# amcpherson/remixt

Measured on AMD Instinct MI355X. Metric: EM iterations/sec (50k seg x 165 states), higher is better.
Workload: dtype f64

## Files before the change

### include/remixt_amd.h

```cpp
#ifndef REMIXT_AMD_H
#define REMIXT_AMD_H

#include <stdint.h>

#ifdef __cplusplus
extern "C" {
#endif

#define RMX_OK 0
#define RMX_EVALUE 1
#define RMX_EASSERT 2
#define RMX_EDEVICE 3
#define RMX_EUNSUPPORTED 4
#define RMX_EARG 5

#define RMX_MAX_CLONES 4

typedef struct rmx_batch rmx_batch;

typedef struct rmx_problem {
    int32_t num_clones;
    int32_t num_segments;
    int32_t num_breakpoints;
    int32_t num_cn_states;
// ... 58 lines not shown
    RMX_OPT_SEARCH_MODE,
    RMX_OPT_ELL_DENSE,
    RMX_OPT_STRIP,
    RMX_OPT_CELL_CACHE,
    RMX_OPT_SPARSE_TRIAL,
    RMX_OPT_FB_DEBUG,
    RMX_OPT_PAIRWISE_KERNEL,
    RMX_OPT_PACE_SWEEPS,
    RMX_OPT_FB_WG_BUDGET,
    RMX_OPT_TRIAL_KERNEL,
    RMX_OPT_GRAD_KERNEL,
    RMX_OPT_STREAM_POOL,
    RMX_OPT_VITERBI_CLUSTER,
    RMX_OPT_TRACEBACK,
    RMX_OPT_LT_CLASSES,
    RMX_OPT_COUNT
};
int rmx_set_default_option(int32_t option_id, int32_t value);
int rmx_set_option(rmx_batch *b, int32_t option_id, int32_t value);
int rmx_get_option(rmx_batch *b, int32_t option_id, int32_t *value);

int rmx_set_param(rmx_batch *b, int32_t r, int32_t param_id, double value);
int rmx_get_param(rmx_batch *b, int32_t r, int32_t param_id, double *value);
int rmx_set_transition_model(rmx_batch *b, int32_t model);
int rmx_set_array(rmx_batch *b, int32_t r, int32_t array_id, const void *host_src);
int rmx_get_array(rmx_batch *b, int32_t r, int32_t array_id, void *host_dst);
int rmx_fetch_indicators(rmx_batch *b, int32_t r0, int32_t r1, const double **total, const double **allele);
int rmx_calculate_log_transmat(rmx_batch *b, int32_t r, double *dst);
int rmx_weighted_search(const double *p, int64_t n, const double *u, int32_t k, int64_t *out, int64_t *positive);
int rmx_weighted_sample_round(const double *w, int64_t n, int64_t stride, double norm, const double *u, int32_t k,
// ... 106 lines not shown
```

### remixt_amd/bpmodel.py

```python
import ctypes as C

import numpy as np

from . import _lib

_dp = C.POINTER(C.c_double)
_ip = C.POINTER(C.c_int64)
_i32p = C.POINTER(C.c_int32)

RMX_EVALUE, RMX_EASSERT, RMX_EDEVICE, RMX_EUNSUPPORTED, RMX_EARG = 1, 2, 3, 4, 5

MAX_CLONES = 4
PARAM_IDS = {
    'negbin_r_0': 0, 'negbin_r_1': 1, 'negbin_hdel_mu': 2, 'negbin_hdel_r_0': 3, 'negbin_hdel_r_1': 4,
    'betabin_M_0': 5, 'betabin_M_1': 6, 'betabin_loh_p': 7, 'betabin_loh_M_0': 8, 'betabin_loh_M_1': 9,
    'prior_outlier_total': 10, 'prior_outlier_allele': 11, 'divergence_weight': 12, 'hmm_log_norm_const': 13,
}
ARRAY_IDS = {
    'h': 0, 'p_breakpoint': 1, 'p_allele_swap': 2, 'p_outlier_total': 3, 'p_outlier_allele': 4,
    'posterior_marginals': 5, 'framelogprob': 6, 'total_likelihood_mask': 7, 'allele_likelihood_mask': 8,
    'log_transmat': 9, 'cached_log_transmat': 10, 'joint_posterior_marginals': 11, 'state_sequence': 12,
}
_WRITABLE = {'h', 'p_breakpoint', 'p_allele_swap', 'p_outlier_total', 'p_outlier_allele', 'posterior_marginals',
             'total_likelihood_mask', 'allele_likelihood_mask'}
_STATE_TABLES = {'cn_states_total': 0, 'num_alleles_subclonal': 1, 'is_hdel': 2, 'is_loh': 3}


OPTION_IDS = dict((n, i) for i, n in enumerate((
    'fb_kernel', 'fb_nv', 'fb_breakend_codes', 'fuse_sweeps', 'two_streams', 'viterbi_plain', 'search_mode', 'ell_dense', 'strip',
    'cell_cache', 'sparse_trial', 'fb_debug', 'pairwise_kernel', 'pace_sweeps', 'fb_wg_budget', 'trial_kernel', 'grad_kernel', 'stream_pool', 'viterbi_cluster', 'traceback', 'lt_classes')))


def set_default_option(name, value):
    lib = _lib.load()
    rc = lib.rmx_set_default_option(OPTION_IDS[name], int(value))
    if rc:
        _raise(lib, rc)


def last_error_restarts():
    lib = _lib.load()
    n = lib.rmx_last_error_restarts(None, 0)
    if n <= 0:
        return []
    buf = (C.c_int32 * n)()
# ... 972 lines not shown
```

### remixt_amd/csrc/rmx_api.hip

```cpp
#include <hip/hip_runtime.h>
#include <algorithm>
#include <cmath>
#include <limits>
#include <atomic>
#include <cstdio>
#include <cstring>
#include <functional>
#include <map>
#include <mutex>
#include <string>
#include <vector>
#include <chrono>
#include <cstdlib>
#include <condition_variable>
#include <memory>

#include "rmx_kernels.h"
#include "rmx_host.h"

static thread_local std::string g_err;
static thread_local std::vector<int32_t> g_err_restarts;
static int fail(int code, const std::string &msg) { g_err = msg; g_err_restarts.clear(); return code; }
static int fail_flagged(int code, const std::string &msg) { g_err = msg; return code; }
static inline long long now_ns() { return std::chrono::duration_cast<std::chrono::nanoseconds>(std::chrono::steady_clock::now().time_since_epoch()).count(); }
// ... 25 lines not shown
    StreamPool &p = g_stream_pool[dev & 15];
    std::lock_guard<std::mutex> lk(p.mu);
    std::vector<hipStream_t> &idle = p.idle[role];
    if (!idle.empty()) { *out = idle.front(); idle.erase(idle.begin()); return RMX_OK; }
    if (hipStreamCreateWithFlags(out, hipStreamNonBlocking) != hipSuccess) return RMX_EDEVICE;
    p.created[role]++;
    return RMX_OK;
}
static void pool_release(int dev, int role, hipStream_t s) {
    hipStreamSynchronize(s);
    StreamPool &p = g_stream_pool[dev & 15];
    std::lock_guard<std::mutex> lk(p.mu);
    p.idle[role].push_back(s);
}

static int g_opt_default[RMX_OPT_COUNT] = {0, 0, 1, 1, 1, 0, 5, 0, 1, 1, 1, 0, 0, 0, 0, 0, 0, 1, 0, 0, 1};
static std::mutex g_opt_mu;

struct rmx_batch {
    hipEvent_t ev_pace = nullptr;
    int opt[RMX_OPT_COUNT];
    int device = 0;
    hipStream_t stream = nullptr;
    hipStream_t stream2 = nullptr;
    hipEvent_t ev_fb = nullptr, ev_brk = nullptr;
    bool own_stream = false, pooled_stream = false, pooled_stream2 = false;
    Dev d{};
    int R = 0;
    std::vector<int64_t> cn_classes;
    std::vector<int32_t> seg_class, brk_idx, brk_orient, tclass, brk_slot, be_n;
    std::vector<int64_t> brk_states, is_telomere;
    std::vector<std::pair<int, int>> tc_pairs;
    std::vector<double> Tsum;
    std::vector<RestartParams> rp;
    std::vector<char> tables_dirty, segc_dirty, ab_dirty;
    std::vector<double> segc_built;
    std::vector<char> sig_valid;
    std::vector<int> cache_stale;
    bool use_cache = false;
    std::vector<int> comp_dirty;
    std::vector<int> comp_base;
    std::vector<int> lt_valid;
    std::vector<int> lt_model, cached_model;
    double *Tval_m[2] = {nullptr, nullptr}; int8_t *af_m[2] = {nullptr, nullptr};
    std::vector<double> plain_T_init;
    std::vector<double> logZ;
    std::vector<char> logz_dirty;
    int *d_lt_valid = nullptr;
    double *d_partial = nullptr;
    double *d_be_e = nullptr;
    double *d_out4 = nullptr;
    double *d_ell_partial = nullptr;
    double *d_ell_out = nullptr;
    double *h_pinned = nullptr;
    hipEvent_t ev_copy = nullptr;
    double *h_ind = nullptr;
// ... 7 lines not shown
    int32_t *d_msample = nullptr, *d_mcounts = nullptr;
    std::vector<int> msample_count;
    double *d_mpartial = nullptr; size_t mpartial_cap = 0;
    std::vector<std::vector<int64_t>> sample_cache; std::vector<int> sample_count;
    double *d_grid_out = nullptr;
    GradFlatLayout gf_lay = {nullptr, nullptr, nullptr, nullptr};
    std::vector<double> gf_sig;
    std::vector<long long> sample_epoch, sig_epoch;
    int32_t *gf_nblk_host = nullptr;
    bool gf_first = false;
    unsigned *d_done = nullptr;
    int32_t *d_rlist = nullptr, *d_counts = nullptr; RestartParams *d_rp_stage = nullptr; double *d_batch_out = nullptr;
    void *h_batch = nullptr;
    std::vector<int32_t> plain_list; int32_t *d_plain_list = nullptr; double *d_plain_jt = nullptr;
    int last_search_blocks = 0;
    unsigned *d_vflag = nullptr; int cluster_timeouts = 0;
    int last_viterbi_wgs = 1;
    int32_t *d_vit_special = nullptr; int n_vit_special = -1;
    double *h_elbo = nullptr; hipEvent_t ev_elbo = nullptr; bool elbo_pending = false, elbo_sync = false; int elbo_r0 = 0, elbo_r1 = 0;
    double *d_vrow = nullptr; size_t vrow_cap = 0;
    uint16_t *d_bp = nullptr; double *d_final = nullptr; int64_t *d_path = nullptr; double *d_logprob = nullptr;
    std::vector<int64_t> last_path; int vit_cap = 0; size_t bp_cap = 0;
    int16_t *d_samp = nullptr; size_t samp_cap = 0; uint64_t *d_seeds = nullptr; uint32_t *d_sflags = nullptr;
    double *d_psum = nullptr; size_t psum_cap = 0; double *d_psw = nullptr; size_t psw_cap = 0;
    double *d_rgcw = nullptr; size_t rgcw_cap = 0;
    double *d_rgn = nullptr; size_t rgn_cap = 0; uint8_t *d_rgt = nullptr; size_t rgt_cap = 0; uint32_t *d_rflags = nullptr; int16_t *d_rgbp = nullptr; size_t rgbp_cap = 0; int kbest_lds_raised = 0;
    double *d_ovr = nullptr; size_t ovr_cap = 0; uint32_t *d_ovf = nullptr; size_t ovf_cap = 0; hipEvent_t ev_ov = nullptr;
    uint16_t *d_comp = nullptr; int32_t *d_ends = nullptr; size_t comp_cap = 0, ends_cap = 0; int last_traceback = 0;
    uint8_t *d_vit_code = nullptr; double *d_vit_val = nullptr; bool vit_code_ok = false, vit_mul_ok = false;
    FbLaunch fbG{}; size_t fbG_lds = 0;
// ... 397 lines not shown
            };
            if (!stale(r)) { r++; continue; }
            int e = r + 1;
            while (e < r1 && stale(e)) e++;
            { ProfScope ps(b, KID_SEG_CONST); hipLaunchKernelGGL(k_seg_const, dim3((b->d.N + 255) / 256, e - r), dim3(256), 0, b->stream, b->d, r); }
            for (int i = r; i < e; i++) b->segc_dirty[i] = 0;
            r = e;
        }
    }
    HIPCHK(hipGetLastError());
    return RMX_OK;
}
typedef void (*cells_kernel_t)(Dev, int);
template <int NS, int LTC> static cells_kernel_t cells_kernel_cached(int mode, int mask, int cache) {
    if (mode == 0) return cache == 2 ? k_cells<NS, 0, CM_ALL, 2, LTC> : k_cells<NS, 0, CM_ALL, 1, LTC>;
    if (mode == 1) return k_cells<NS, 1, CM_ALL, 2, LTC>;
    if (mode == 3) return k_cells<NS, 3, CM_ALL, 2, LTC>;
    if (cache == 2) return k_cells<NS, 2, 31, 2, LTC>;
    switch (mask) {
    case 1: return k_cells<NS, 2, 1, 1, LTC>; case 2: return k_cells<NS, 2, 2, 1, LTC>;
    case 3: return k_cells<NS, 2, 3, 1, LTC>; case 4: return k_cells<NS, 2, 4, 1, LTC>; case 8: return k_cells<NS, 2, 8, 1, LTC>;
    case 12: return k_cells<NS, 2, 12, 1, LTC>; case 15: return k_cells<NS, 2, 15, 1, LTC>; default: return k_cells<NS, 2, 31, 1, LTC>;
    }
}
template <int NS> static cells_kernel_t cells_kernel_ns(int mode, int mask, int cache, bool ltc) {
    if (cache) return ltc ? cells_kernel_cached<NS, 1>(mode, mask, cache) : cells_kernel_cached<NS, 0>(mode, mask, cache);
    if (mode == 0) return k_cells<NS, 0, CM_ALL, 0, 0>;
    if (mode == 1) return k_cells<NS, 1, CM_ALL, 0, 0>;
    switch (mask) {
    case 1: return k_cells<NS, 2, 1, 0, 0>; case 2: return k_cells<NS, 2, 2, 0, 0>;
    case 3: return k_cells<NS, 2, 3, 0, 0>; case 4: return k_cells<NS, 2, 4, 0, 0>; case 8: return k_cells<NS, 2, 8, 0, 0>;
    case 12: return k_cells<NS, 2, 12, 0, 0>; case 15: return k_cells<NS, 2, 15, 0, 0>; default: return k_cells<NS, 2, 31, 0, 0>;
    }
}
static bool use_strip(rmx_batch *b) { return b->d.S > 32 && b->d.S <= 384 && b->opt[RMX_OPT_STRIP]; }
static cells_kernel_t cells_kernel(rmx_batch *b, int mode, int mask, int cache) {
    const int ns = (b->d.S + 63) / 64;
    const bool ltc = cache != 0 && b->d.ltc != nullptr;
    switch (ns) { case 1: return cells_kernel_ns<1>(mode, mask, cache, ltc); case 2: return cells_kernel_ns<2>(mode, mask, cache, ltc);
                  case 3: return cells_kernel_ns<3>(mode, mask, cache, ltc); case 4: return cells_kernel_ns<4>(mode, mask, cache, ltc);
                  case 5: return cells_kernel_ns<5>(mode, mask, cache, ltc); default: return cells_kernel_ns<6>(mode, mask, cache, ltc); }
}
// ... 537 lines not shown
    HIPCHK(hipHostMalloc(&b->h_batch, (size_t)R * (sizeof(RestartParams) + 64) + 4096));
    HIPCHK(hipEventCreate(&b->tm_a)); HIPCHK(hipEventCreate(&b->tm_b));
    b->done_ev.resize(R);
    for (int r = 0; r < R; r++) HIPCHK(hipEventCreateWithFlags(&b->done_ev[r], hipEventDisableTiming));

    if ((rc = build_transitions(b))) { rmx_batch_destroy(b); return rc; }
    {
        double tmin = 0.;
        std::vector<double> tv((size_t)SS * d.TC);
        if (d.TC) HIPCHK(hipMemcpy(tv.data(), d.Tval, tv.size() * 8, hipMemcpyDeviceToHost));
        for (double v : tv) tmin = std::min(tmin, v);
        if (tmin < -650.) { rmx_batch_destroy(b); return fail(RMX_EUNSUPPORTED, "transition_log_prob * max copy-number change exceeds 650 nats: outside the linear-domain envelope"); }
    }

    b->sample_cache.assign(R, std::vector<int64_t>()); b->sample_count.assign(R, -1);
    b->rp.resize(R); b->tables_dirty.assign(R, 1); b->segc_dirty.assign(R, 1); b->ab_dirty.assign(R, 1); b->comp_dirty.assign(R, 31); b->comp_base.assign(R, 31); b->cache_stale.assign(R, 15); b->sig_valid.assign(R, 0); b->sample_epoch.assign(R, 0); b->sig_epoch.assign(R, 0); b->lt_valid.assign(R, 0); b->lt_model.assign(R, 0); b->cached_model.assign(R, 0); b->logZ.assign(R, 0.); b->logz_dirty.assign(R, 0);
    for (int r = 0; r < R; r++) {
        RestartParams &p = b->rp[r];
        memset(&p, 0, sizeof p);
        for (int m = 0; m < M; m++) p.h[m] = h_init[(size_t)r * M + m];
        p.p[RMX_P_NEGBIN_R_0] = 500.; p.p[RMX_P_NEGBIN_R_1] = 10.; p.p[RMX_P_NEGBIN_HDEL_MU] = 1e-5; p.p[RMX_P_NEGBIN_HDEL_R_0] = 10.;
        p.p[RMX_P_NEGBIN_HDEL_R_1] = 1.; p.p[RMX_P_BETABIN_M_0] = 500.; p.p[RMX_P_BETABIN_M_1] = 10.; p.p[RMX_P_BETABIN_LOH_P] = 1e-3;
        p.p[RMX_P_BETABIN_LOH_M_0] = 10.; p.p[RMX_P_BETABIN_LOH_M_1] = 1.; p.p[RMX_P_PRIOR_OUTLIER_TOTAL] = 0.01; p.p[RMX_P_PRIOR_OUTLIER_ALLELE] = 0.01;
        p.p[RMX_P_DIVERGENCE_WEIGHT] = std::fabs(divw[r]);
    }
    {
        std::vector<double> q2(RN * 2), v;
        for (size_t i = 0; i < RN; i++) { q2[2 * i] = 1. - 0.01; q2[2 * i + 1] = 0.01; }
        HIPCHK(hipMemcpy(d.qt, q2.data(), q2.size() * 8, hipMemcpyHostToDevice));
        HIPCHK(hipMemcpy(d.qa, q2.data(), q2.size() * 8, hipMemcpyHostToDevice));
        for (size_t i = 0; i < RN * 2; i++) q2[i] = 0.5;
// ... 64 lines not shown
    else { HIPCHK(hipStreamCreateWithFlags(&b->stream, hipStreamNonBlocking)); b->own_stream = true; }
    return RMX_OK;
}
int rmx_synchronize(rmx_batch *b) { BIND(b); HIPCHK(hipStreamSynchronize(b->stream)); return RMX_OK; }

int rmx_info(rmx_batch *b, int32_t what, int64_t *out) { BIND(b);
    switch (what) {
    case 0: *out = b->d.cn_max; break; case 1: *out = b->d.NC; break; case 2: *out = b->d.TC; break; case 3: *out = b->d.NBE; break;
    case 4: *out = b->d.SP; break; case 5: *out = b->fbv_rpt; break; case 6: *out = b->fbG.P; break; case 7: *out = b->fbG.NT; break;
    case 8: *out = b->fbG.BLK; break; case 9: *out = (int64_t)b->fbG_lds; break; case 10: *out = b->n_fast; break; case 11: *out = b->n_generic; break;
    case 60: *out = b->t_launch_ns; break; case 61: *out = b->t_wait_ns; break; case 62: *out = b->t_post_ns; break; case 63: *out = b->n_rounds; break;
    case 12: *out = b->last_fb_kernel; break; case 13: *out = b->last_fb_nv; break; case 14: *out = b->last_viterbi; break; case 15: *out = b->last_fb_nv_max; break;
    case 18: *out = b->last_viterbi_wgs; break; case 19: *out = b->last_traceback; break;
    case 64: *out = b->d.NT; break; case 65: *out = b->d.ltc ? 1 : 0; break;
    case 54: *out = b->cluster_timeouts; break;
    case 52: *out = b->last_search_blocks; break;
    case 16: { StreamPool &p_ = g_stream_pool[b->device & 15]; std::lock_guard<std::mutex> lk(p_.mu); *out = p_.created[0] + p_.created[1]; break; }
    case 17: { StreamPool &p_ = g_stream_pool[b->device & 15]; std::lock_guard<std::mutex> lk(p_.mu); *out = (int64_t)(p_.idle[0].size() + p_.idle[1].size()); break; }
    case 20: case 21: case 22: case 23: case 24: case 25: case 26: case 27: case 28: case 29: case 30: case 31: case 32: case 33: case 34: case 35: case 36: case 37: case 38: case 39:
    case 40: case 41: case 42: case 43: case 44: case 45: case 46: case 47: case 48: case 49: case 50: case 51:
        { if (!b->d_dbg) { *out = 0; break; } unsigned long long v[32]; HIPCHK(hipStreamSynchronize(b->stream)); HIPCHK(hipMemcpy(v, b->d_dbg, 256, hipMemcpyDeviceToHost)); *out = (int64_t)v[what - 20]; break; }
    default: return fail(RMX_EARG, "bad info id");
    }
    return RMX_OK;
}

static const int kParamComponents[RMX_P_HMM_LOG_NORM_CONST] = {CM_LT0, CM_LT1, CM_LT0 | CM_LT1, CM_LT0, CM_LT1, CM_LA0, CM_LA1, CM_LA0 | CM_LA1, CM_LA0, CM_LA1, 0, 0, 16};
int rmx_set_param(rmx_batch *b, int32_t r, int32_t id, double v) { BIND(b);
    if (r < 0 || r >= b->R || id < 0 || id >= RMX_P_HMM_LOG_NORM_CONST) return fail(RMX_EARG, "bad restart / param id");
    if (id == RMX_P_DIVERGENCE_WEIGHT) v = std::fabs(v);
// ... 24 lines not shown

static int array_shape(rmx_batch *b, int id, size_t *count, bool *is_int) {
    const Dev &d = b->d; *is_int = false;
    switch (id) {
    case RMX_A_H: *count = d.M; break;
    case RMX_A_P_BREAKPOINT: *count = (size_t)d.K * d.B; break;
    case RMX_A_P_ALLELE_SWAP: case RMX_A_P_OUTLIER_TOTAL: case RMX_A_P_OUTLIER_ALLELE: *count = (size_t)d.N * 2; break;
    case RMX_A_POSTERIOR_MARGINALS: case RMX_A_FRAMELOGPROB: *count = (size_t)d.N * d.S; break;
    case RMX_A_TOTAL_LIKELIHOOD_MASK: case RMX_A_ALLELE_LIKELIHOOD_MASK: case RMX_A_STATE_SEQUENCE: *count = d.N; *is_int = true; break;
    case RMX_A_LOG_TRANSMAT: case RMX_A_CACHED_LOG_TRANSMAT: case RMX_A_JOINT_POSTERIOR_MARGINALS: *count = (size_t)(d.N - 1) * d.S * d.S; break;
    default: return fail(RMX_EARG, "bad array id");
    }
    return RMX_OK;
}

int rmx_set_array(rmx_batch *b, int32_t r, int32_t id, const void *src) { BIND(b);
    if (r < 0 || r >= b->R || !src) return fail(RMX_EARG, "bad restart / null source");
    Dev &d = b->d;
    const size_t RN = (size_t)r * d.N;
    switch (id) {
    case RMX_A_H:
        for (int m = 0; m < d.M; m++) b->rp[r].h[m] = ((const double *)src)[m];
        b->tables_dirty[r] = 1; b->ab_dirty[r] = 1; b->comp_dirty[r] = 31; b->comp_base[r] = 31; b->cache_stale[r] = 15; return RMX_OK;
    case RMX_A_P_BREAKPOINT:
        if (d.K) HIPCHK(hipMemcpyAsync(d.pbrk + (size_t)r * d.K * d.B, src, (size_t)d.K * d.B * 8, hipMemcpyHostToDevice, b->stream));
        break;
    case RMX_A_P_ALLELE_SWAP: HIPCHK(hipMemcpyAsync(d.qs + RN * 2, src, (size_t)d.N * 16, hipMemcpyHostToDevice, b->stream)); break;
    case RMX_A_P_OUTLIER_TOTAL: HIPCHK(hipMemcpyAsync(d.qt + RN * 2, src, (size_t)d.N * 16, hipMemcpyHostToDevice, b->stream)); break;
    case RMX_A_P_OUTLIER_ALLELE: HIPCHK(hipMemcpyAsync(d.qa + RN * 2, src, (size_t)d.N * 16, hipMemcpyHostToDevice, b->stream)); break;
    case RMX_A_POSTERIOR_MARGINALS:
        HIPCHK(hipMemcpy2DAsync(d.post + RN * d.SP, (size_t)d.SP * 8, src, (size_t)d.S * 8, (size_t)d.S * 8, d.N, hipMemcpyHostToDevice, b->stream));
        b->ab_dirty[r] = 1; b->comp_dirty[r] = 31; b->comp_base[r] = 31; b->sig_valid[r] = 0; b->sig_epoch[r]++; break;
    case RMX_A_TOTAL_LIKELIHOOD_MASK: case RMX_A_ALLELE_LIKELIHOOD_MASK: {
        std::vector<uint8_t> m8(d.N);
        for (int n = 0; n < d.N; n++) m8[n] = ((const int64_t *)src)[n] != 0;
        HIPCHK(hipStreamSynchronize(b->stream));
        HIPCHK(hipMemcpy((void *)(id == RMX_A_TOTAL_LIKELIHOOD_MASK ? d.mask_t : d.mask_a), m8.data(), d.N, hipMemcpyHostToDevice));
        for (int i = 0; i < b->R; i++) { b->ab_dirty[i] = 1; b->comp_dirty[i] = 31; b->comp_base[i] = 31; b->cache_stale[i] = 15; }
        return RMX_OK; }
    default: return fail(RMX_EARG, "array is read-only or unknown");
    }
    HIPCHK(hipStreamSynchronize(b->stream));
    return RMX_OK;
}

int rmx_get_array(rmx_batch *b, int32_t r, int32_t id, void *dst) { BIND(b);
    if (r < 0 || r >= b->R || !dst) return fail(RMX_EARG, "bad restart / null destination");
    Dev &d = b->d;
    const size_t RN = (size_t)r * d.N;
    switch (id) {
    case RMX_A_H: for (int m = 0; m < d.M; m++) ((double *)dst)[m] = b->rp[r].h[m]; return RMX_OK;
    case RMX_A_P_BREAKPOINT: if (d.K) HIPCHK(hipMemcpyAsync(dst, d.pbrk + (size_t)r * d.K * d.B, (size_t)d.K * d.B * 8, hipMemcpyDeviceToHost, b->stream)); break;
    case RMX_A_P_ALLELE_SWAP: HIPCHK(hipMemcpyAsync(dst, d.qs + RN * 2, (size_t)d.N * 16, hipMemcpyDeviceToHost, b->stream)); break;
// ... 99 lines not shown
        for (int s = 0; s < S; s++) {
            if (which == 0) { for (int m = 0; m < M; m++) dst[((size_t)n * S + s) * M + m] = t[(s * M + m) * 2] + t[(s * M + m) * 2 + 1]; continue; }
            bool hdel = true, loh = false; int nsub = 0;
            for (int m = 0; m < M; m++) if (t[(s * M + m) * 2] || t[(s * M + m) * 2 + 1]) hdel = false;
            for (int a = 0; a < 2; a++) {
                int64_t sum = 0; for (int m = 0; m < M; m++) sum += t[(s * M + m) * 2 + a];
                if (sum == 0) loh = true;
                if (M > 1) { int64_t lo = t[(s * M + 1) * 2 + a], hi = lo; for (int m = 2; m < M; m++) { lo = std::min(lo, t[(s * M + m) * 2 + a]); hi = std::max(hi, t[(s * M + m) * 2 + a]); } if (hi != lo) nsub++; }
            }
            dst[(size_t)n * S + s] = which == 1 ? nsub : (which == 2 ? (hdel ? 1 : 0) : (loh ? 1 : 0));
        }
    }
    return RMX_OK;
}

static int do_framelogprob(rmx_batch *b, int r0, int r1) {
    int rc = ensure_tables(b, r0, r1);
    if (rc) return rc;
    ProfScope ps(b, KID_FRAMELOGPROB);
    if (use_strip(b)) {
        int r = r0;
        while (r < r1) {
            const bool cur = b->use_cache && b->cache_stale[r] == 0;
            int e = r;
            while (e < r1 && (b->use_cache && b->cache_stale[e] == 0) == cur) e++;
            hipLaunchKernelGGL(cells_kernel(b, 0, CM_ALL, cur ? 2 : (b->use_cache ? 1 : 0)), strip_grid(b, e - r), dim3(256), 0, b->stream, b->d, r);
            if (b->use_cache) for (int i = r; i < e; i++) b->cache_stale[i] = 0;
            r = e;
        }
    }
    else hipLaunchKernelGGL(k_framelogprob, row_grid(b, r1 - r0), dim3(256), 0, b->stream, b->d, r0, b->G);
    HIPCHK(hipGetLastError());
    return RMX_OK;
}
static inline int fb_wg_budget(const rmx_batch *b) { return b->opt[RMX_OPT_FB_WG_BUDGET] > 0 ? b->opt[RMX_OPT_FB_WG_BUDGET] : b->num_cus; }
static void (*fbm_kernel_for(int KB))(FbmArgs) {
    switch (KB) { case 8: return k_fbm<8>; case 16: return k_fbm<16>; case 28: return k_fbm<28>; case 36: return k_fbm<36>; case 42: return k_fbm<42>; case 44: return k_fbm<44>; }
    return nullptr;
}
static int fb_items_for(rmx_batch *b, int r0, int r1, int pin, const double (&cost)[5], rmx_batch::FbItems **out) {
    if ((pin == 1 || pin == 2 || pin == 4) && cost[pin] == 0.) pin = 4;
// ... 27 lines not shown
    std::vector<int4> items;
    rmx_batch::FbItems f;
    for (int c : order) {
        const int nv = nv_of[c];
        f.nv_min = std::min(f.nv_min, nv); f.nv_max = std::max(f.nv_max, nv);
        for (int u = r0 / nv; u <= (r1 - 1) / nv; u++) for (int dir = 0; dir < 2; dir++) items.push_back(make_int4(b->h_list_fast[c], u * nv, nv, dir));
    }
    f.n = (int)items.size();
    int rc = dalloc(b, &f.dev, items.size());
    if (rc) return rc;
    HIPCHK(hipMemcpy(f.dev, items.data(), items.size() * sizeof(int4), hipMemcpyHostToDevice));
    *out = &(b->fb_items[key] = f);
    return RMX_OK;
}
static int p_cn_front(rmx_batch *b, int r0, int r1, bool skip_frame, bool snapshot_done = false) {
    int rc = skip_frame ? ensure_tables(b, r0, r1) : do_framelogprob(b, r0, r1);
    if (rc) return rc;
    if (!snapshot_done && (rc = launch_brk_lut(b, r0, r1, b->d.pd_lt, b->d.pe_lt))) return rc;
    {
        ProfScope ps(b, KID_FB);
        const Dev &d = b->d;
        FbArgs a;
        a.S = d.S; a.SP = d.SP; a.M = d.M; a.D = d.D; a.C = d.C; a.N = d.N; a.NBE = d.NBE; a.cn_max = d.cn_max;
        a.r0 = r0; a.pen = d.pen;
        a.chain_start = d.chain_start; a.chain_end = d.chain_end; a.tclass = d.tclass; a.brk_slot = d.brk_slot;
        a.chain_tc = d.chain_tc; a.chain_cls = d.chain_cls; a.be_cls = d.be_cls; a.amat_lds = 0; a.pad_ = 0;
        a.fe = d.fe; a.Wf = d.Wf; a.Wb = d.Wb; a.pe_lt = d.pe_lt; a.af = d.af; a.ab = d.ab; a.tot = d.tot;
        a.fa = d.fa; a.fb = d.fb; a.mrow = d.mrow; a.err = d.err; a.dbg = b->d_dbg;
        bool fast = false;
        bool done_fast = false;
        if (b->fbv_rpt > 0 && b->n_fast > 0 && d.M <= 3 && (d.NBE == 0 || (d.pe2x_lt != nullptr && b->max_adist < 64 && b->opt[RMX_OPT_FB_BREAKEND_CODES])) &&
// ... 132 lines not shown
        }
        HIPCHK(hipGetLastError());
    }
    for (int r = r0; r < r1; r++) b->lt_model[r] = b->d.tmodel;
    for (int r = r0; r < r1; r++) { if (!b->lt_valid[r]) { b->lt_valid[r] = 1; int one = 1; HIPCHK(hipMemcpyAsync(b->d_lt_valid + r, &one, 4, hipMemcpyHostToDevice, b->stream)); } }
    return RMX_OK;
}
static int p_cn_marginals(rmx_batch *b, int r0, int r1, bool fuse_next) {
    {
        ProfScope ps(b, KID_MARGINALS);
        if (use_strip(b)) hipLaunchKernelGGL(cells_kernel(b, fuse_next ? 3 : 1, CM_ALL, b->use_cache ? 2 : 0), strip_grid(b, r1 - r0), dim3(256), 0, b->stream, b->d, r0);
        else hipLaunchKernelGGL(k_marginals<true>, row_grid(b, r1 - r0), dim3(256), 0, b->stream, b->d, r0, b->G);
        HIPCHK(hipGetLastError());
    }
    if (fuse_next && use_strip(b)) std::swap(b->d.fe, b->d.fe_alt);
    for (int r = r0; r < r1; r++) { b->ab_dirty[r] = 0; b->comp_dirty[r] = 0; b->comp_base[r] = 0; b->logz_dirty[r] = 1; b->sig_valid[r] = (!fuse_next && use_strip(b) && b->d.sig_cnt) ? 1 : 0; b->sig_epoch[r]++; }
    return RMX_OK;
}
static int do_update_p_cn(rmx_batch *b, int r0, int r1, bool skip_frame = false, bool fuse_next = false) {
    int rc;
    if ((rc = p_cn_front(b, r0, r1, skip_frame)) || (rc = launch_pairwise_breakends(b, r0, r1, 0))) return rc;
    return p_cn_marginals(b, r0, r1, fuse_next);
}
static int do_update_p_breakpoint(rmx_batch *b, int r0, int r1, bool snapshot = false) {
    const Dev &d = b->d;
    if (d.K > 0 && d.NBE > 0) {
        ProfScope ps(b, KID_BRK_UPDATE);
        hipLaunchKernelGGL(k_brk_update_lut, dim3(d.K, r1 - r0), dim3(128), (size_t)d.B * 16, b->stream, b->d, r0, b->d.pd_cached,
                           snapshot ? b->d.pd_lt : (double *)nullptr, b->d.pe_lt, b->d.pe2_lt, b->pe2p);
        HIPCHK(hipGetLastError());
    } else {
// ... 9 lines not shown
    const double pti = plain_T_mean_sum(b);
    for (int r = r0; r < r1; r++) { b->plain_T_init[r] = pti; b->cached_model[r] = b->d.tmodel; }
    return RMX_OK;
}
static int do_indicator(rmx_batch *b, int r0, int r1, int which) {
    int rc = ensure_ab(b, r0, r1);
    if (rc) return rc;
    dim3 g((b->d.N + 255) / 256, r1 - r0);
    if (which == 0) { ProfScope ps(b, KID_OUTLIER_TOTAL); hipLaunchKernelGGL(k_update_outlier_total, g, dim3(256), 0, b->stream, b->d, r0); }
    else if (which == 1) { ProfScope ps(b, KID_OUTLIER_ALLELE); hipLaunchKernelGGL(k_update_outlier_allele, g, dim3(256), 0, b->stream, b->d, r0); }
    else { ProfScope ps(b, KID_ALLELE_SWAP); hipLaunchKernelGGL(k_update_allele_swap, g, dim3(256), 0, b->stream, b->d, r0); }
    HIPCHK(hipGetLastError());
    return RMX_OK;
}

int rmx_update_framelogprob(rmx_batch *b, int32_t r0, int32_t r1) { BIND(b); RANGE_CHECK(); int rc = do_framelogprob(b, r0, r1); return rc ? rc : check_errors(b, r0, r1); }
int rmx_update_p_cn(rmx_batch *b, int32_t r0, int32_t r1) { BIND(b); RANGE_CHECK(); int rc = do_update_p_cn(b, r0, r1); return rc ? rc : check_errors(b, r0, r1); }
int rmx_update_p_breakpoint(rmx_batch *b, int32_t r0, int32_t r1) { BIND(b); RANGE_CHECK(); int rc = do_update_p_breakpoint(b, r0, r1); return rc ? rc : check_errors(b, r0, r1); }
int rmx_update_p_outlier_total(rmx_batch *b, int32_t r0, int32_t r1) { BIND(b); RANGE_CHECK(); int rc = do_indicator(b, r0, r1, 0); return rc ? rc : check_errors(b, r0, r1); }
int rmx_update_p_outlier_allele(rmx_batch *b, int32_t r0, int32_t r1) { BIND(b); RANGE_CHECK(); int rc = do_indicator(b, r0, r1, 1); return rc ? rc : check_errors(b, r0, r1); }
int rmx_update_p_allele_swap(rmx_batch *b, int32_t r0, int32_t r1) { BIND(b); RANGE_CHECK(); int rc = do_indicator(b, r0, r1, 2); return rc ? rc : check_errors(b, r0, r1); }

int rmx_variational_update(rmx_batch *b, int32_t r0, int32_t r1, int32_t iters) { BIND(b);
    RANGE_CHECK();
    const bool fusable = use_strip(b) && b->use_cache && b->opt[RMX_OPT_FUSE_SWEEPS];
    const bool two_streams = use_strip(b) && b->d.NBE > 0 && b->opt[RMX_OPT_TWO_STREAMS];
    if (two_streams && !b->stream2) {
        if (b->opt[RMX_OPT_STREAM_POOL]) { if (pool_acquire(b->device, 1, &b->stream2) != RMX_OK) return fail(RMX_EDEVICE, "hipStreamCreate failed"); b->pooled_stream2 = true; }
        else HIPCHK(hipStreamCreateWithFlags(&b->stream2, hipStreamNonBlocking));
        HIPCHK(hipEventCreateWithFlags(&b->ev_fb, hipEventDisableTiming));
        HIPCHK(hipEventCreateWithFlags(&b->ev_brk, hipEventDisableTiming));
// ... 771 lines not shown
    HIPCHK(hipGetLastError());
    HIPCHK(hipMemcpyAsync(b->h_pinned, b->d_out4, (size_t)nr * 8, hipMemcpyDeviceToHost, b->stream));
    if ((rc = check_errors(b, r0, r1))) return rc;
    for (int i = 0; i < nr; i++) out[i] = b->h_pinned[i];
    return RMX_OK;
}

static int trial_pass(rmx_batch *b, int r0, int r1, Dev &d2) {
    b->trial_comp_r0 = b->trial_comp_r1 = -1;
    b->scratch_r0 = b->scratch_r1 = -1;
    int rc = ensure_tables(b, r0, r1);
    if (rc) return rc;
    const Dev &d = b->d;
    const int nr = r1 - r0;
    const size_t RN0 = (size_t)r0 * d.N, cnt = (size_t)nr * d.N;
    HIPCHK(hipMemcpyAsync(b->d_A2 + RN0 * 2, d.A + RN0 * 2, cnt * 16, hipMemcpyDeviceToDevice, b->stream));
    HIPCHK(hipMemcpyAsync(b->d_Bv2 + RN0 * 4, d.Bv + RN0 * 4, cnt * 32, hipMemcpyDeviceToDevice, b->stream));
    d2 = b->d;
    d2.A = b->d_A2; d2.Bv = b->d_Bv2; d2.lc = nullptr; d2.ltc = nullptr;
    for (int r = r0; r < r1;) {
        const int mask = use_strip(b) ? cover_mask(b->comp_dirty[r] & 15) : (b->comp_dirty[r] ? 15 : 0);
        int e = r + 1;
        while (e < r1 && (use_strip(b) ? cover_mask(b->comp_dirty[e] & 15) : (b->comp_dirty[e] ? 15 : 0)) == mask) e++;
        if (mask) {
            ProfScope ps(b, KID_MARGINALS_AB);
            bool sparse = use_strip(b) && d.sig_cnt != nullptr;
            for (int i = r; i < e; i++) if (!b->sig_valid[i]) sparse = false;
            if (sparse) {
                void (*kf)(Dev, int) = nullptr;
                if (b->opt[RMX_OPT_TRIAL_KERNEL] == 0) {
                    switch (mask) {
                    case 1: kf = k_trial_flat<1>; break; case 2: kf = k_trial_flat<2>; break; case 3: kf = k_trial_flat<3>; break;
                    case 4: kf = k_trial_flat<4>; break; case 8: kf = k_trial_flat<8>; break; case 12: kf = k_trial_flat<12>; break;
                    default: kf = k_trial_flat<15>; break;
                    }
                    hipLaunchKernelGGL(kf, dim3((d.N + TF_SEGB - 1) / TF_SEGB, e - r), dim3(256), 0, b->stream, d2, r);
                } else {
                    switch (mask) {
// ... 929 lines not shown
```

### remixt_amd/csrc/rmx_kernels.h

```cpp
#pragma once
#include "rmx_device.h"
#include "rmx_host.h"
#define SEGL 32
#define SEG_PER_BLOCK (256 / SEGL)
#define TRIAL_SEGL 16
#define RMX_CLUSTER_SPINS (1u << 22)
#define FBK_WKN 128
#define NM_MAX_SAMPLE 1024
#define TRIAL_SEG_PER_BLOCK (256 / TRIAL_SEGL)


__device__ __forceinline__ void state_tables_body(const Dev &d, int cls, int r, const RestartParams &rp) {
    __shared__ unsigned agg_sh;
    if (threadIdx.x == 0) agg_sh = 0u;
    __syncthreads();
    unsigned agg = 0u;
    for (int s = threadIdx.x; s < d.S; s += blockDim.x) {
        const int8_t *cn = d.cn + ((size_t)cls * d.S + s) * d.M * 2;
        const int8_t *tot = d.tot + ((size_t)cls * d.S + s) * d.M;
        double minor = 0., total = 0.;
        for (int m = 0; m < d.M; m++) {
            minor += rp.h[m] * (double)cn[m * 2 + 0];
            total += rp.h[m] * (double)tot[m];
        }
// ... 1703 lines not shown
#pragma unroll
                for (int j = 0; j < 2; j++) {
                    const int kc = lane + 64 * j;
                    if ((j == 0 || d.NT > 64) && kc < d.NT) {
                        StateRegs rs_ = {};
                        rs_.D = repD[LTG && CACHE == 1 ? j : 0]; rs_.logD = repLogD[LTG && CACHE == 1 ? j : 0]; rs_.fl = repFl[LTG && CACHE == 1 ? j : 0];
                        double LTc[2], LAc[4];
                        cell_ll_regs<MASK & (CM_LT0 | CM_LT1)>(rp, sc, rs_, LTc, LAc, err);
                        if (LTG0) { ltr[lo_ + kc] = LTc[0]; ltl[wave][kc] = LTc[0]; }
                        if (LTG1) { ltr[lplane + lo_ + kc] = LTc[1]; ltl[wave][128 + kc] = LTc[1]; }
                    }
                }
            }
            __builtin_amdgcn_wave_barrier();
        };
        if (MODE == 0) {
            const double qt0 = d.qt[rn * 2], qt1 = d.qt[rn * 2 + 1], qa0 = d.qa[rn * 2], qa1 = d.qa[rn * 2 + 1];
            const double qs0 = d.qs[rn * 2], qs1 = d.qs[rn * 2 + 1];
            double fv[NS];
            double vmax = -INFINITY;
            lt_rows_to_lds();
#pragma unroll
            for (int k = 0; k < NS; k++) {
                const int s = lane + 64 * k;
                fv[k] = -INFINITY;
                if (s < S) {
                    double LT[2], LA[4];
                    cell(sc, st[k], (size_t)n * d.SP + s, k, LT, LA);
                    double f = 0.;
                    f += qt0 * LT[0]; f += qt1 * LT[1];
                    f += qa0 * qs0 * LA[0]; f += qa0 * qs1 * LA[1]; f += qa1 * qs0 * LA[2]; f += qa1 * qs1 * LA[3];
                    f += -1.0 * (CACHE == 2 ? nsub_of(cls, s) : st[k].nsub) * sc.l * divw;
                    if (f != f) err |= RMX_ERR_NAN_F;
                    d.f[ro + s] = f;
                    fv[k] = f;
                    vmax = fmax(vmax, f);
                }
                __builtin_amdgcn_sched_barrier(0);
            }
            vmax = group_max(vmax, 64);
            if (lane == 0) d.fmax[rn] = vmax;
#pragma unroll
            for (int k = 0; k < NS; k++) { const int s = lane + 64 * k; if (s < d.SP) d.fe[ro + s] = s < S ? exp_fast(fv[k] - vmax) : 0.; }
        } else {
            constexpr bool M1 = MODE == 1 || MODE == 3;
            constexpr int LAOFF = LTC ? 0 : 2;
            constexpr int NSTASH = MODE != 3 ? 0 : LTC ? (NS <= 3 ? 4 : (NS == 4 ? 3 : 2)) : (NS <= 3 ? 6 : (NS <= 6 ? 3 : 0));
            constexpr bool STASH = NSTASH > 0;
            __shared__ double lsm[STASH ? 4 : 1][STASH ? NS * NSTASH * 64 : 1];
// ... 5233 lines not shown
```

Before: 456.1.

## Skip redundant frame stores, trial buffer copies, and f-dependent refreshes

Adds a cells kernel mode 4 that computes frame log-probs and the exp-normalised values but does not write the raw f array. It is used when a marginal pass follows immediately. It also skips the device-to-device copies of A and Bv into the trial buffers when every restart's launch mask rewrites all components. When h or the likelihood masks change and the frame was not moved externally, it narrows the dirty component mask from 31 to 15. Together these cut global memory writes and copies per EM iteration, at the cost of extra bookkeeping (f_moved) and a risk of stale f values or trial buffers if a later path still reads them.

```diff
diff --git a/include/remixt_amd.h b/include/remixt_amd.h
--- a/include/remixt_amd.h
+++ b/include/remixt_amd.h
@@ -96,6 +96,9 @@
     RMX_OPT_VITERBI_CLUSTER,
     RMX_OPT_TRACEBACK,
     RMX_OPT_LT_CLASSES,
+    RMX_OPT_FRAME_STORE,
+    RMX_OPT_PF_REFRESH,
+    RMX_OPT_TRIAL_COPY,
     RMX_OPT_COUNT
 };
 int rmx_set_default_option(int32_t option_id, int32_t value);
diff --git a/remixt_amd/bpmodel.py b/remixt_amd/bpmodel.py
--- a/remixt_amd/bpmodel.py
+++ b/remixt_amd/bpmodel.py
@@ -28,7 +28,8 @@
 
 OPTION_IDS = dict((n, i) for i, n in enumerate((
     'fb_kernel', 'fb_nv', 'fb_breakend_codes', 'fuse_sweeps', 'two_streams', 'viterbi_plain', 'search_mode', 'ell_dense', 'strip',
-    'cell_cache', 'sparse_trial', 'fb_debug', 'pairwise_kernel', 'pace_sweeps', 'fb_wg_budget', 'trial_kernel', 'grad_kernel', 'stream_pool', 'viterbi_cluster', 'traceback', 'lt_classes')))
+    'cell_cache', 'sparse_trial', 'fb_debug', 'pairwise_kernel', 'pace_sweeps', 'fb_wg_budget', 'trial_kernel', 'grad_kernel', 'stream_pool', 'viterbi_cluster', 'traceback', 'lt_classes',
+    'frame_store', 'pf_refresh', 'trial_copy')))
 
 
 def set_default_option(name, value):
diff --git a/remixt_amd/csrc/rmx_api.hip b/remixt_amd/csrc/rmx_api.hip
--- a/remixt_amd/csrc/rmx_api.hip
+++ b/remixt_amd/csrc/rmx_api.hip
@@ -63,7 +63,7 @@
     p.idle[role].push_back(s);
 }
 
-static int g_opt_default[RMX_OPT_COUNT] = {0, 0, 1, 1, 1, 0, 5, 0, 1, 1, 1, 0, 0, 0, 0, 0, 0, 1, 0, 0, 1};
+static int g_opt_default[RMX_OPT_COUNT] = {0, 0, 1, 1, 1, 0, 5, 0, 1, 1, 1, 0, 0, 0, 0, 0, 0, 1, 0, 0, 1, 0, 0, 0};
 static std::mutex g_opt_mu;
 
 struct rmx_batch {
@@ -89,6 +89,7 @@
     bool use_cache = false;
     std::vector<int> comp_dirty;
     std::vector<int> comp_base;
+    std::vector<char> f_moved;
     std::vector<int> lt_valid;
     std::vector<int> lt_model, cached_model;
     double *Tval_m[2] = {nullptr, nullptr}; int8_t *af_m[2] = {nullptr, nullptr};
@@ -126,6 +127,7 @@
     void *h_batch = nullptr;
     std::vector<int32_t> plain_list; int32_t *d_plain_list = nullptr; double *d_plain_jt = nullptr;
     int last_search_blocks = 0;
+    bool last_trial_copied = false;
     unsigned *d_vflag = nullptr; int cluster_timeouts = 0;
     int last_viterbi_wgs = 1;
     int32_t *d_vit_special = nullptr; int n_vit_special = -1;
@@ -553,6 +555,7 @@
 typedef void (*cells_kernel_t)(Dev, int);
 template <int NS, int LTC> static cells_kernel_t cells_kernel_cached(int mode, int mask, int cache) {
     if (mode == 0) return cache == 2 ? k_cells<NS, 0, CM_ALL, 2, LTC> : k_cells<NS, 0, CM_ALL, 1, LTC>;
+    if (mode == 4) return cache == 2 ? k_cells<NS, 4, CM_ALL, 2, LTC> : k_cells<NS, 4, CM_ALL, 1, LTC>;
     if (mode == 1) return k_cells<NS, 1, CM_ALL, 2, LTC>;
     if (mode == 3) return k_cells<NS, 3, CM_ALL, 2, LTC>;
     if (cache == 2) return k_cells<NS, 2, 31, 2, LTC>;
@@ -565,6 +568,7 @@
 template <int NS> static cells_kernel_t cells_kernel_ns(int mode, int mask, int cache, bool ltc) {
     if (cache) return ltc ? cells_kernel_cached<NS, 1>(mode, mask, cache) : cells_kernel_cached<NS, 0>(mode, mask, cache);
     if (mode == 0) return k_cells<NS, 0, CM_ALL, 0, 0>;
+    if (mode == 4) return k_cells<NS, 4, CM_ALL, 0, 0>;
     if (mode == 1) return k_cells<NS, 1, CM_ALL, 0, 0>;
     switch (mask) {
     case 1: return k_cells<NS, 2, 1, 0, 0>; case 2: return k_cells<NS, 2, 2, 0, 0>;
@@ -1132,7 +1136,7 @@
     }
 
     b->sample_cache.assign(R, std::vector<int64_t>()); b->sample_count.assign(R, -1);
-    b->rp.resize(R); b->tables_dirty.assign(R, 1); b->segc_dirty.assign(R, 1); b->ab_dirty.assign(R, 1); b->comp_dirty.assign(R, 31); b->comp_base.assign(R, 31); b->cache_stale.assign(R, 15); b->sig_valid.assign(R, 0); b->sample_epoch.assign(R, 0); b->sig_epoch.assign(R, 0); b->lt_valid.assign(R, 0); b->lt_model.assign(R, 0); b->cached_model.assign(R, 0); b->logZ.assign(R, 0.); b->logz_dirty.assign(R, 0);
+    b->rp.resize(R); b->tables_dirty.assign(R, 1); b->segc_dirty.assign(R, 1); b->ab_dirty.assign(R, 1); b->comp_dirty.assign(R, 31); b->comp_base.assign(R, 31); b->f_moved.assign(R, 0); b->cache_stale.assign(R, 15); b->sig_valid.assign(R, 0); b->sample_epoch.assign(R, 0); b->sig_epoch.assign(R, 0); b->lt_valid.assign(R, 0); b->lt_model.assign(R, 0); b->cached_model.assign(R, 0); b->logZ.assign(R, 0.); b->logz_dirty.assign(R, 0);
     for (int r = 0; r < R; r++) {
         RestartParams &p = b->rp[r];
         memset(&p, 0, sizeof p);
@@ -1227,6 +1231,7 @@
     case 18: *out = b->last_viterbi_wgs; break; case 19: *out = b->last_traceback; break;
     case 64: *out = b->d.NT; break; case 65: *out = b->d.ltc ? 1 : 0; break;
     case 54: *out = b->cluster_timeouts; break;
+    case 66: *out = b->last_trial_copied ? 1 : 0; break;
     case 52: *out = b->last_search_blocks; break;
     case 16: { StreamPool &p_ = g_stream_pool[b->device & 15]; std::lock_guard<std::mutex> lk(p_.mu); *out = p_.created[0] + p_.created[1]; break; }
     case 17: { StreamPool &p_ = g_stream_pool[b->device & 15]; std::lock_guard<std::mutex> lk(p_.mu); *out = (int64_t)(p_.idle[0].size() + p_.idle[1].size()); break; }
@@ -1281,6 +1286,7 @@
     return RMX_OK;
 }
 
+static int h_components(const rmx_batch *b, int r) { return (b->opt[RMX_OPT_PF_REFRESH] || b->f_moved[r]) ? 31 : 15; }
 int rmx_set_array(rmx_batch *b, int32_t r, int32_t id, const void *src) { BIND(b);
     if (r < 0 || r >= b->R || !src) return fail(RMX_EARG, "bad restart / null source");
     Dev &d = b->d;
@@ -1288,7 +1294,7 @@
     switch (id) {
     case RMX_A_H:
         for (int m = 0; m < d.M; m++) b->rp[r].h[m] = ((const double *)src)[m];
-        b->tables_dirty[r] = 1; b->ab_dirty[r] = 1; b->comp_dirty[r] = 31; b->comp_base[r] = 31; b->cache_stale[r] = 15; return RMX_OK;
+        b->tables_dirty[r] = 1; b->ab_dirty[r] = 1; b->comp_dirty[r] = h_components(b, r) | (b->comp_dirty[r] & 16); b->comp_base[r] = h_components(b, r) | (b->comp_base[r] & 16); b->cache_stale[r] = 15; return RMX_OK;
     case RMX_A_P_BREAKPOINT:
         if (d.K) HIPCHK(hipMemcpyAsync(d.pbrk + (size_t)r * d.K * d.B, src, (size_t)d.K * d.B * 8, hipMemcpyHostToDevice, b->stream));
         break;
@@ -1303,7 +1309,7 @@
         for (int n = 0; n < d.N; n++) m8[n] = ((const int64_t *)src)[n] != 0;
         HIPCHK(hipStreamSynchronize(b->stream));
         HIPCHK(hipMemcpy((void *)(id == RMX_A_TOTAL_LIKELIHOOD_MASK ? d.mask_t : d.mask_a), m8.data(), d.N, hipMemcpyHostToDevice));
-        for (int i = 0; i < b->R; i++) { b->ab_dirty[i] = 1; b->comp_dirty[i] = 31; b->comp_base[i] = 31; b->cache_stale[i] = 15; }
+        for (int i = 0; i < b->R; i++) { b->ab_dirty[i] = 1; b->comp_dirty[i] = h_components(b, i) | (b->comp_dirty[i] & 16); b->comp_base[i] = h_components(b, i) | (b->comp_base[i] & 16); b->cache_stale[i] = 15; }
         return RMX_OK; }
     default: return fail(RMX_EARG, "array is read-only or unknown");
     }
@@ -1433,7 +1439,8 @@
     return RMX_OK;
 }
 
-static int do_framelogprob(rmx_batch *b, int r0, int r1) {
+static int do_framelogprob(rmx_batch *b, int r0, int r1, bool marginal_follows = false) {
+    const int fmode = marginal_follows && !b->opt[RMX_OPT_FRAME_STORE] ? 4 : 0;
     int rc = ensure_tables(b, r0, r1);
     if (rc) return rc;
     ProfScope ps(b, KID_FRAMELOGPROB);
@@ -1443,7 +1450,7 @@
             const bool cur = b->use_cache && b->cache_stale[r] == 0;
             int e = r;
             while (e < r1 && (b->use_cache && b->cache_stale[e] == 0) == cur) e++;
-            hipLaunchKernelGGL(cells_kernel(b, 0, CM_ALL, cur ? 2 : (b->use_cache ? 1 : 0)), strip_grid(b, e - r), dim3(256), 0, b->stream, b->d, r);
+            hipLaunchKernelGGL(cells_kernel(b, fmode, CM_ALL, cur ? 2 : (b->use_cache ? 1 : 0)), strip_grid(b, e - r), dim3(256), 0, b->stream, b->d, r);
             if (b->use_cache) for (int i = r; i < e; i++) b->cache_stale[i] = 0;
             r = e;
         }
@@ -1501,7 +1508,7 @@
     return RMX_OK;
 }
 static int p_cn_front(rmx_batch *b, int r0, int r1, bool skip_frame, bool snapshot_done = false) {
-    int rc = skip_frame ? ensure_tables(b, r0, r1) : do_framelogprob(b, r0, r1);
+    int rc = skip_frame ? ensure_tables(b, r0, r1) : do_framelogprob(b, r0, r1, true);
     if (rc) return rc;
     if (!snapshot_done && (rc = launch_brk_lut(b, r0, r1, b->d.pd_lt, b->d.pe_lt))) return rc;
     {
@@ -1664,7 +1671,7 @@
         HIPCHK(hipGetLastError());
     }
     if (fuse_next && use_strip(b)) std::swap(b->d.fe, b->d.fe_alt);
-    for (int r = r0; r < r1; r++) { b->ab_dirty[r] = 0; b->comp_dirty[r] = 0; b->comp_base[r] = 0; b->logz_dirty[r] = 1; b->sig_valid[r] = (!fuse_next && use_strip(b) && b->d.sig_cnt) ? 1 : 0; b->sig_epoch[r]++; }
+    for (int r = r0; r < r1; r++) { b->ab_dirty[r] = 0; b->comp_dirty[r] = 0; b->comp_base[r] = 0; b->f_moved[r] = 0; b->logz_dirty[r] = 1; b->sig_valid[r] = (!fuse_next && use_strip(b) && b->d.sig_cnt) ? 1 : 0; b->sig_epoch[r]++; }
     return RMX_OK;
 }
 static int do_update_p_cn(rmx_batch *b, int r0, int r1, bool skip_frame = false, bool fuse_next = false) {
@@ -1704,7 +1711,7 @@
     return RMX_OK;
 }
 
-int rmx_update_framelogprob(rmx_batch *b, int32_t r0, int32_t r1) { BIND(b); RANGE_CHECK(); int rc = do_framelogprob(b, r0, r1); return rc ? rc : check_errors(b, r0, r1); }
+int rmx_update_framelogprob(rmx_batch *b, int32_t r0, int32_t r1) { BIND(b); RANGE_CHECK(); int rc = do_framelogprob(b, r0, r1); for (int r = r0; r < r1; r++) b->f_moved[r] = 1; return rc ? rc : check_errors(b, r0, r1); }
 int rmx_update_p_cn(rmx_batch *b, int32_t r0, int32_t r1) { BIND(b); RANGE_CHECK(); int rc = do_update_p_cn(b, r0, r1); return rc ? rc : check_errors(b, r0, r1); }
 int rmx_update_p_breakpoint(rmx_batch *b, int32_t r0, int32_t r1) { BIND(b); RANGE_CHECK(); int rc = do_update_p_breakpoint(b, r0, r1); return rc ? rc : check_errors(b, r0, r1); }
 int rmx_update_p_outlier_total(rmx_batch *b, int32_t r0, int32_t r1) { BIND(b); RANGE_CHECK(); int rc = do_indicator(b, r0, r1, 0); return rc ? rc : check_errors(b, r0, r1); }
@@ -2506,14 +2513,20 @@
     const Dev &d = b->d;
     const int nr = r1 - r0;
     const size_t RN0 = (size_t)r0 * d.N, cnt = (size_t)nr * d.N;
-    HIPCHK(hipMemcpyAsync(b->d_A2 + RN0 * 2, d.A + RN0 * 2, cnt * 16, hipMemcpyDeviceToDevice, b->stream));
-    HIPCHK(hipMemcpyAsync(b->d_Bv2 + RN0 * 4, d.Bv + RN0 * 4, cnt * 32, hipMemcpyDeviceToDevice, b->stream));
+    auto launch_mask = [&](int r) { return use_strip(b) ? cover_mask(b->comp_dirty[r] & 15) : (b->comp_dirty[r] ? 15 : 0); };
+    bool all_written = !b->opt[RMX_OPT_TRIAL_COPY];
+    for (int r = r0; r < r1 && all_written; r++) all_written = launch_mask(r) == 15;
+    if (!all_written) {
+        HIPCHK(hipMemcpyAsync(b->d_A2 + RN0 * 2, d.A + RN0 * 2, cnt * 16, hipMemcpyDeviceToDevice, b->stream));
+        HIPCHK(hipMemcpyAsync(b->d_Bv2 + RN0 * 4, d.Bv + RN0 * 4, cnt * 32, hipMemcpyDeviceToDevice, b->stream));
+    }
+    b->last_trial_copied = !all_written;
     d2 = b->d;
     d2.A = b->d_A2; d2.Bv = b->d_Bv2; d2.lc = nullptr; d2.ltc = nullptr;
     for (int r = r0; r < r1;) {
-        const int mask = use_strip(b) ? cover_mask(b->comp_dirty[r] & 15) : (b->comp_dirty[r] ? 15 : 0);
+        const int mask = launch_mask(r);
         int e = r + 1;
-        while (e < r1 && (use_strip(b) ? cover_mask(b->comp_dirty[e] & 15) : (b->comp_dirty[e] ? 15 : 0)) == mask) e++;
+        while (e < r1 && launch_mask(e) == mask) e++;
         if (mask) {
             ProfScope ps(b, KID_MARGINALS_AB);
             bool sparse = use_strip(b) && d.sig_cnt != nullptr;
diff --git a/remixt_amd/csrc/rmx_kernels.h b/remixt_amd/csrc/rmx_kernels.h
--- a/remixt_amd/csrc/rmx_kernels.h
+++ b/remixt_amd/csrc/rmx_kernels.h
@@ -1741,7 +1741,7 @@
             }
             __builtin_amdgcn_wave_barrier();
         };
-        if (MODE == 0) {
+        if (MODE == 0 || MODE == 4) {
             const double qt0 = d.qt[rn * 2], qt1 = d.qt[rn * 2 + 1], qa0 = d.qa[rn * 2], qa1 = d.qa[rn * 2 + 1];
             const double qs0 = d.qs[rn * 2], qs1 = d.qs[rn * 2 + 1];
             double fv[NS];
@@ -1759,7 +1759,7 @@
                     f += qa0 * qs0 * LA[0]; f += qa0 * qs1 * LA[1]; f += qa1 * qs0 * LA[2]; f += qa1 * qs1 * LA[3];
                     f += -1.0 * (CACHE == 2 ? nsub_of(cls, s) : st[k].nsub) * sc.l * divw;
                     if (f != f) err |= RMX_ERR_NAN_F;
-                    d.f[ro + s] = f;
+                    if (MODE == 0) d.f[ro + s] = f;
                     fv[k] = f;
                     vmax = fmax(vmax, f);
                 }
```

After: 444.2. 2.6% lower.
